# nianticlabs/map-free-reloc

Measured on AMD Instinct MI355X. Metric: image-pairs/sec @ 540x720 (SuperPoint+SuperGlue + PnP w/ depth), higher is better.
Workload: dtype f32 in / f32 accumulate; matrix products of the 3x3 convolutions, attention, the transformer's linear layers and SuperPoint's 1x1 descriptor head on the f16 matrix cores with every fp32 operand carried as TWO f16 terms (xh = rne_f16(x), xl = rne_f16((x - xh) 2^11); weights pre-scaled per output feat

## Files before the change

include/mfr_hip.h:

```cpp
#ifndef MFR_HIP_H
#define MFR_HIP_H
#include <stddef.h>
#include <stdint.h>

#ifdef __cplusplus
extern "C" {
#endif

#define MFR_ABI_VERSION 6

#define MFR_K_F32 0
#define MFR_K_F64 1

#define MFR_E_ARG      (-1)
#define MFR_E_LAUNCH   (-2)
#define MFR_E_WORKSPACE (-3)

#define MFR_ST_OK          0
#define MFR_ST_TOO_FEW     1
#define MFR_ST_BAD_DEPTH   2
#define MFR_ST_NO_MODEL    3
#define MFR_ST_DEGENERATE  4

int mfr_abi_version(void);
// ... 193 lines not shown
int mfr_sift_detect(const uint8_t *gray, int B, int H, int W, int nfeatures, int Nmax, int cand_cap, void *workspace,
                    size_t workspace_bytes, float *kpts, float *desc, float *size, float *angle, float *response,
                    int32_t *octave, int32_t *n, int32_t *status, void *stream);

size_t mfr_jpeg_workspace_bytes(int n, int H, int W, long long max_record_bytes, int subseq_bits);
int mfr_jpeg_decode(const void *headers, const uint8_t *records, const long long *offsets, int n, int H, int W,
                    long long max_record_bytes, float *gray, uint8_t *rgb, int32_t *status, int32_t *rounds, void *workspace,
                    size_t workspace_bytes, int subseq_bits, void *stream);

int mfr_resize_gray_bilinear(const uint8_t *rgb, int n, int H, int W, const int32_t *status,
                             const int32_t *y0, const int32_t *y1, const float *fy,
                             const int32_t *x0, const int32_t *x1, const float *fx,
                             int h, int w, float *out, void *stream);

size_t mfr_wino_f16x2_filter_bytes(int Cin, int Cout);
int mfr_wino_f16x2_filter_transform(const float *w, int Cin, int Cout, void *upk, void *stream);
int mfr_conv3x3_wino_f16x2(const float *x, const void *upk, const float *bias, const float *residual, int B, int Cin, int Cout,
                           int H, int W, int act, int pool, float *y, void *stream);
size_t mfr_conv3x3_direct_f16x2_filter_bytes(int Cin, int Cout);
int mfr_conv3x3_direct_f16x2_filter_pack(const float *w, int Cin, int Cout, void *packed, void *stream);
int mfr_conv3x3_direct_f16x2(const float *x, const void *packed, const float *bias, const float *residual, int B, int Cin, int Cout,
                             int H, int W, int act, int pool, float *y, void *stream);
int mfr_conv3x3_direct_f16x2_rows(const float *x, const void *packed, const float *bias, int B, int Cin, int Cout, int H, int W, int act, float *yrows, int ldy, void *stream);
int mfr_conv3x3s2_direct_f16x2(const float *x, const void *packed, const float *bias, int B, int Cin, int Cout, int H, int W, int act, float *y, void *stream);
int mfr_sp_conv1ab_f16x2(const float *gray, const float *w1a, const float *b1a, const void *upk1b, const float *bias1b, int B, int H, int W, float *y, void *stream);
size_t mfr_wino_bf16x3_filter_bytes(int Cin, int Cout);
int mfr_wino_bf16x3_filter_transform(const float *w, int Cin, int Cout, void *upk, void *stream);
int mfr_conv3x3_wino_bf16x3(const float *x, const void *upk, const float *bias, const float *residual, int B, int Cin, int Cout,
                            int H, int W, int act, int pool, float *y, void *stream);
size_t mfr_wino_filter_bytes(int Cin, int Cout);
int mfr_wino_filter_transform(const float *w, int Cin, int Cout, float *upk, void *stream);
int mfr_conv3x3_wino(const float *x, const float *upk, const float *bias, const float *residual, int B, int Cin, int Cout,
                     int H, int W, int act, int pool, float *y, void *stream);
int mfr_conv3x3_wino_variant(const float *x, const float *upk, const float *bias, const float *residual, int B, int Cin, int Cout,
                             int H, int W, int act, int pool, int variant, float *y, void *stream);

int mfr_corr_warp_fwd(const float *q, const float *k, const float *v, const float *grid, int B, int Dq, int N,
                      float *warped, float *pos, float *max_score, float *row_max, float *row_sum, void *stream);
int mfr_corr_warp_bwd(const float *q, const float *k, const float *v, const float *grid, int B, int Dq, int N,
                      const float *d_warped, const float *d_pos, const float *d_max, const float *delta,
                      const float *row_max, const float *row_sum, float *dq, float *dk, float *dv, void *stream);

#ifdef __cplusplus
}
#endif
#endif
// ... 1 lines not shown
```

map-free-reloc_amd/_lib.py:

```python
import ctypes as C
import os

_HERE = os.path.dirname(os.path.abspath(__file__))
SO_PATH = os.path.join(_HERE, "csrc", "libmfr_hip.so")

_lib = None

_vp, _i, _d, _u64, _sz = C.c_void_p, C.c_int, C.c_double, C.c_uint64, C.c_size_t

SIGNATURES = {
    "mfr_abi_version": (_i, []),
    "mfr_target_arch": (C.c_char_p, []),
    "mfr_f16x2_guard_bind": (_i, [_vp]),
    "mfr_test_f64_ops": (_i, [_vp, _vp, _vp, _i, _vp, _vp]),
    "mfr_test_sample": (_i, [_u64, _vp, _i, _i, _i, _i, _vp, _vp]),
    "mfr_pnp_workspace_bytes": (_sz, [_i, _i, _i]),
    "mfr_pnp_solve_batch": (_i, [_vp, _vp, _vp, _i, _i, _vp, _i, _i, _vp, _vp, _i, _i, _d, _d, _u64, _vp,
                                 _vp, _sz, _vp, _vp, _vp, _vp, _vp, _vp]),
    "mfr_depth_min": (_i, [_vp, _i, _i, _i, _vp, _vp]),
    "mfr_pnp_lift": (_i, [_vp, _vp, _vp, _i, _i, _vp, _vp, _i, _i, _vp, _i, _vp, _vp, _vp, _vp, _vp]),
    "mfr_pnp_ransac": (_i, [_vp, _vp, _vp, _i, _i, _vp, _i, _i, _d, _d, _u64, _vp, _vp, _vp, _vp, _vp, _vp, _vp,
                            _vp, _vp, _vp, _vp]),
    "mfr_emat_workspace_bytes": (_sz, [_i, _i, _i]),
    "mfr_magsac_lut": (_i, [_vp, _i]),
# ... 39 lines not shown
    "mfr_loftr_ot_match_workspace_bytes": (_sz, [_i, _i, _i]),
    "mfr_loftr_ot_match": (_i, [_vp, _i, _i, _i, _i, _i, C.c_float, _i, C.c_float, _i, _vp, _sz, _vp, _vp, _vp, _vp, _vp, _vp, _i, _vp]),
    "mfr_loftr_coarse_match_variant": (_i, [_vp, _i, _i, _i, _i, _i, C.c_float, C.c_float, _i, _vp, _sz, _vp, _vp, _vp, _vp, _i, _vp]),
    "mfr_loftr_fine_attention": (_i, [_vp, _i, _vp, _vp, _i, _i, _i, _i, _i, _vp, _i, _vp]),
    "mfr_loftr_gather_windows": (_i, [_vp, _i, _i, _i, _i, _vp, _vp, _i, _i, _i, _i, _vp, _vp]),
    "mfr_loftr_fine_match": (_i, [_vp, _vp, _i, _i, _i, _i, C.c_float, _vp, _vp, _vp, _vp, _vp]),
    "mfr_conv3x3_c1_relu": (_i, [_vp, _vp, _vp, _i, _i, _i, _i, _vp, _vp]),
    "mfr_bias_relu_nchw": (_i, [_vp, _vp, _i, _i, _i, _vp]),
    "mfr_conv1x1_nchw": (_i, [_vp, _vp, _vp, _i, _i, _i, _i, _vp, _vp]),
    "mfr_nchw_to_rows": (_i, [_vp, _vp, _i, _i, _i, _i, _vp, C.c_longlong, _i, _vp]),
    "mfr_bias_pool2_relu_nchw": (_i, [_vp, _vp, _i, _i, _i, _i, _vp, _vp]),
    "mfr_wino_bf16x3_filter_bytes": (_sz, [_i, _i]),
    "mfr_wino_bf16x3_filter_transform": (_i, [_vp, _i, _i, _vp, _vp]),
    "mfr_conv3x3_wino_bf16x3": (_i, [_vp, _vp, _vp, _vp, _i, _i, _i, _i, _i, _i, _i, _vp, _vp]),
    "mfr_sp_conv1ab_f16x2": (_i, [_vp, _vp, _vp, _vp, _vp, _i, _i, _i, _vp, _vp]),
    "mfr_wino_f16x2_filter_bytes": (_sz, [_i, _i]),
    "mfr_wino_f16x2_filter_transform": (_i, [_vp, _i, _i, _vp, _vp]),
    "mfr_conv3x3_wino_f16x2": (_i, [_vp, _vp, _vp, _vp, _i, _i, _i, _i, _i, _i, _i, _vp, _vp]),
    "mfr_conv3x3_direct_f16x2_filter_bytes": (_sz, [_i, _i]),
    "mfr_conv3x3_direct_f16x2_filter_pack": (_i, [_vp, _i, _i, _vp, _vp]),
    "mfr_conv3x3_direct_f16x2": (_i, [_vp, _vp, _vp, _vp, _i, _i, _i, _i, _i, _i, _i, _vp, _vp]),
    "mfr_conv3x3s2_direct_f16x2": (_i, [_vp, _vp, _vp, _i, _i, _i, _i, _i, _i, _vp, _vp]),
    "mfr_conv3x3_direct_f16x2_rows": (_i, [_vp, _vp, _vp, _i, _i, _i, _i, _i, _i, _vp, _i, _vp]),
    "mfr_wino_filter_bytes": (_sz, [_i, _i]),
    "mfr_wino_filter_transform": (_i, [_vp, _i, _i, _vp, _vp]),
    "mfr_conv3x3_wino": (_i, [_vp, _vp, _vp, _vp, _i, _i, _i, _i, _i, _i, _i, _vp, _vp]),
    "mfr_conv3x3_wino_variant": (_i, [_vp, _vp, _vp, _vp, _i, _i, _i, _i, _i, _i, _i, _i, _vp, _vp]),
    "mfr_layernorm": (_i, [_vp, _i, _vp, _vp, _vp, _i, C.c_longlong, _i, C.c_float, _vp, _i, _vp]),
    "mfr_conv_gemm_bf16": (_i, [_vp, C.c_longlong, _vp, _vp, C.c_longlong, _vp, _i, _i, _i, _vp, _vp, C.c_longlong, _i,
                                _i, _i, _i, _vp, _vp, _vp, _vp, _vp]),
    "mfr_conv_pack_nhwc_halo": (_i, [_vp, _i, _i, _i, _i, _i, _i, _vp, _i, _vp]),
    "mfr_conv_unpack_nchw": (_i, [_vp, _i, _i, _i, _i, _i, _vp, _vp]),
    "mfr_conv_pack_cm_halo": (_i, [_vp, _i, C.c_longlong, _i, _i, _i, C.c_longlong, _i, _i, C.c_longlong, _vp, _vp]),
    "mfr_upsample2x_add": (_i, [_vp, _vp, _i, _i, _i, _vp]),
    "mfr_upsample_bilinear": (_i, [_vp, _vp, _i, _i, _i, _i, _i, _i, _vp]),
    "mfr_corr_warp_fwd": (_i, [_vp, _vp, _vp, _vp, _i, _i, _i, _vp, _vp, _vp, _vp, _vp, _vp]),
    "mfr_corr_warp_bwd": (_i, [_vp, _vp, _vp, _vp, _i, _i, _i, _vp, _vp, _vp, _vp, _vp, _vp, _vp, _vp, _vp, _vp]),
    "mfr_kabsch_fwd": (_i, [_vp, _i, _vp, _vp]),
    "mfr_kabsch_bwd": (_i, [_vp, _vp, _i, _vp, _vp]),
    "mfr_rootsift": (_i, [_vp, _i, _vp, _vp, _vp]),
    "mfr_desc_ratio_match": (_i, [_vp, _vp, _vp, _vp, _vp, _vp, _i, _i, _i, _vp, _vp, _d, _vp, _vp, _vp, _vp, _i, _vp, _vp]),
    "mfr_sift_workspace_bytes": (_sz, [_i, _i, _i, _i]),
    "mfr_sift_level_offset": (C.c_longlong, [_i, _i, _i, _i, _i, _vp, _vp]),
    "mfr_sift_blur_taps": (_i, [_i, _vp, _vp]),
    "mfr_sift_detect": (_i, [_vp, _i, _i, _i, _i, _i, _i, _vp, _sz, _vp, _vp, _vp, _vp, _vp, _vp, _vp, _vp, _vp]),
    "mfr_jpeg_workspace_bytes": (_sz, [_i, _i, _i, C.c_longlong, _i]),
# ... 55 lines not shown
```

map-free-reloc_amd/csrc/conv_direct.hip:

```cpp
#include <hip/hip_runtime.h>
#include <stdint.h>
#include <type_traits>

#include "../../include/mfr_hip.h"
#include "wave_dev.h"
#include "split_f16.h"
#include "guard.h"

using namespace mfr;

typedef float dc_f32x16 __attribute__((ext_vector_type(16)));
#define DC_OOB 0x80000000u
#define DC_PC 34
#define DC_FRAGS_PER_TAP 6
#ifndef DC_NW
#define DC_NW 4
#endif

#ifdef DC_PROF
__device__ unsigned long long dc_prof[8][64];
#define DC_STAMP(k) do { if (blockIdx.x == (gridDim.x / 2 | 5u) && lane == 0) { __builtin_amdgcn_sched_barrier(0); dc_prof[w][(k)] = __builtin_amdgcn_s_memtime(); __builtin_amdgcn_sched_barrier(0); } } while (0)
extern "C" int *mfr_guard_current(void) { return nullptr; }
#else
#define DC_STAMP(k) do { } while (0)
#endif

#define DC_IC(k) std::integral_constant<int, k>{}
template <int MG, int NW, int STR> struct DcGeom {
    static constexpr int NT = 64 * NW;
    static constexpr int NGW = NW / MG;
    static constexpr int TR = 4 * NGW;
    static constexpr int PR = STR == 1 ? TR + 2 : 2 * TR + 1;
    static constexpr int PCW = STR == 1 ? DC_PC : 66;
    static constexpr int P = PR * PCW;
    static constexpr int PPAD = (P + 63) / 64 * 64;
    static constexpr int STAGE = 4 * PPAD;
    static constexpr int R = (2 * PPAD + NT - 1) / NT;
};

__global__ void __launch_bounds__(64) dc_scale_kernel(const float *__restrict__ w, int Cin, int Cout, int cpad, float *__restrict__ oscale)
{
    const int co = blockIdx.x, lane = threadIdx.x;
    float mx = 0.f;
    if (co < Cout)
        for (int t = lane; t < Cin * 9; t += 64) mx = fmaxf(mx, fabsf(w[(size_t)co * Cin * 9 + t]));
    mx = wave_max(mx);
    if (lane == 0 && co < cpad) oscale[co] = 1.0f / sf_feature_scale(mx);
}
__global__ void __launch_bounds__(256) dc_pack_kernel(const float *__restrict__ w, int Cin, int Cout, int nks, long long total, const float *__restrict__ oscale, uint4 *__restrict__ out)
{
    const long long t = (long long)blockIdx.x * 256 + threadIdx.x;
    if (t >= total) return;
    const int l = (int)(t & 63);
    long long f = t >> 6;
    const int term = (int)(f % 3); f /= 3;
    const int m = (int)(f & 1); f >>= 1;
    const int tap = (int)(f % 9); f /= 9;
    const int c = (int)(f % nks);
    const int cg = (int)(f / nks);
    const int co = cg * 64 + m * 32 + (l & 31);
    const float s = 1.0f / oscale[co];
    unsigned short hw[8];
#pragma unroll
    for (int e = 0; e < 8; ++e) {
        const int ci = 16 * c + 8 * (l >> 5) + e;
        const float v = (co < Cout && ci < Cin) ? w[((size_t)co * Cin + ci) * 9 + tap] * s : 0.f;
        unsigned short wh, wl, wq;
        sf_split_w(v, wh, wl, wq);
        hw[e] = term == 0 ? wh : term == 1 ? wl : wq;
    }
    out[t] = make_uint4((unsigned)hw[0] | ((unsigned)hw[1] << 16), (unsigned)hw[2] | ((unsigned)hw[3] << 16),
                        (unsigned)hw[4] | ((unsigned)hw[5] << 16), (unsigned)hw[6] | ((unsigned)hw[7] << 16));
}

template <int MG, int NW, bool POOL, int STR>
__global__ void __launch_bounds__(64 * NW, 8 / NW) conv_direct_f16x2_kernel(
    const float *__restrict__ x, const uint4 *__restrict__ wp, unsigned wp_bytes, const float *__restrict__ oscale, const float *__restrict__ bias,
    const float *__restrict__ residual, float *__restrict__ y, int Cin, int Cout, int H, int W, int nbx, int nby, int S, int ncgw, int nks, int act, int *guard, int ldrows)
{
    static_assert(STR == 1 || (STR == 2 && !POOL), "stride 1 or 2; no pooled strided variant");
    using G = DcGeom<MG, NW, STR>;
    __shared__ __attribute__((aligned(16))) uint4 lds[2 * G::STAGE];
    const int tid = threadIdx.x, lane = tid & 63;
    const int w = __builtin_amdgcn_readfirstlane(tid >> 6);
    const int xcd = blockIdx.x & 7, slot = blockIdx.x >> 3;
    const int cgi = slot % ncgw, s = (slot / ncgw) * 8 + xcd;
    if (s >= S) return;
    const int bx = s % nbx, by = (s / nbx) % nby, b = s / (nbx * nby);
    const int x0 = 32 * bx, y0 = G::TR * by;
    const int HW = H * W;
    const int Hout = STR == 1 ? H : (H - 1) / 2 + 1, Wout = STR == 1 ? W : (W - 1) / 2 + 1;
    const bool tail = !POOL && NW == 4 && MG == 2 && cgi == ncgw - 1 && (Cout - cgi * 128 + 31) / 32 == 3;

    const __amdgpu_buffer_rsrc_t rsX = __builtin_amdgcn_make_buffer_rsrc((void *)(x + (size_t)b * Cin * HW), 0, Cin * HW * 4, MFR_RSRC_FLAGS);
    unsigned voff[G::R];
    int wdst[G::R], hh[G::R];
#pragma unroll
    for (int r = 0; r < G::R; ++r) {
        const int h = (G::NT * r + 64 * w) / G::PPAD;
        const int p = G::NT * r + tid - h * G::PPAD;
        const int pr = p / G::PCW, q = p - pr * G::PCW;
        const int pc = STR == 1 ? q : 2 * (q % 33) + q / 33;
        const int gy = STR * y0 - 1 + pr, gx = STR * x0 - 1 + pc;
        const bool ok = h < 2 && p < G::P && pc < STR * 32 + 3 - STR && gy >= 0 && gy < H && gx >= 0 && gx < W;
        voff[r] = ok ? (unsigned)(gy * W + gx) * 4u : DC_OOB;
        hh[r] = h < 2 ? h : 0;
        wdst[r] = h < 2 ? h * G::PPAD + p : G::P + (lane & 15);
    }
    float sv[8];
    auto sload = [&](int r, int c) {
#pragma unroll
        for (int e = 0; e < 8; ++e) {
            const int ch = 16 * c + 8 * hh[r] + e;
            sv[e] = __builtin_bit_cast(float, __builtin_amdgcn_raw_buffer_load_b32(rsX, ch < Cin ? voff[r] : DC_OOB, (unsigned)ch * (unsigned)HW * 4u, 0));
        }
    };
    auto swrite = [&](int r, int buf) {
        unsigned h[4], l[4];
#pragma unroll
        for (int k = 0; k < 4; ++k) sf_split2(sv[2 * k], sv[2 * k + 1], SF_LOW_SCALE, h[k], l[k]);
        lds[buf * G::STAGE + wdst[r]] = make_uint4(h[0], h[1], h[2], h[3]);
        lds[buf * G::STAGE + 2 * G::PPAD + wdst[r]] = make_uint4(l[0], l[1], l[2], l[3]);
    };

    const __amdgpu_buffer_rsrc_t rsW = __builtin_amdgcn_make_buffer_rsrc((void *)wp, 0, (int)wp_bytes, MFR_RSRC_FLAGS);
    const unsigned lane16 = (unsigned)lane * 16u;
    auto body = [&](auto mbc, auto nbc) {
    constexpr int MB = decltype(mbc)::value, NB = decltype(nbc)::value;
    const int mg = MB == 2 ? w % MG : 0, ng = MB == 2 ? w / MG : w;
    const int mb0 = (cgi * MG + mg) * 2;
    const unsigned kstride = (unsigned)nks * (9u * DC_FRAGS_PER_TAP * 1024u);
    auto aload = [&](int c, int tap, int m, int term) -> uint4 {
        const int mbg = mb0 + m;
        return __builtin_bit_cast(uint4, __builtin_amdgcn_raw_buffer_load_b128(rsW, lane16, (unsigned)(mbg >> 1) * kstride + (unsigned)(((c * 9 + tap) * 2 + (mbg & 1)) * 3 + term) * 1024u, 0));
    };
    const int rdb = (lane >> 5) * G::PPAD + (STR * NB * ng) * G::PCW + (lane & 31);
    auto tapoff = [](int n, int dy, int dx) { return STR == 1 ? (n + dy) * G::PCW + dx : (2 * n + dy) * G::PCW + (dx & 1) * 33 + (dx >> 1); };

    DC_STAMP(0);
    {
        float pv[G::R][8];
#pragma unroll
        for (int r = 0; r < G::R; ++r) { sload(r, 0);
#pragma unroll
            for (int e = 0; e < 8; ++e) pv[r][e] = sv[e]; }
#pragma unroll
        for (int r = 0; r < G::R; ++r) {
#pragma unroll
            for (int e = 0; e < 8; ++e) sv[e] = pv[r][e];
            swrite(r, 0); }
    }
    uint4 AE[MB][3], AO[MB][3], Bh[NB], Bl[NB];
#pragma unroll
    for (int m = 0; m < MB; ++m) { AE[m][0] = aload(0, 0, m, 0); AE[m][1] = aload(0, 0, m, 1); AE[m][2] = aload(0, 0, m, 2); AO[m][1] = aload(0, 1, m, 1); AO[m][2] = aload(0, 1, m, 2); AO[m][0] = AE[m][0]; }
    dc_f32x16 acc[MB][NB];
#pragma unroll
    for (int m = 0; m < MB; ++m)
#pragma unroll
        for (int n = 0; n < NB; ++n)
#pragma unroll
            for (int r = 0; r < 16; ++r) acc[m][n][r] = 0.f;

#define DC_SL(r) (G::R == 5 ? 5 * (r) : 8 * (r))
#define DC_SW(r) (G::R == 5 ? ((r) == 4 ? 26 : 5 * (r) + 4) : ((r) == 2 ? 24 : 8 * (r) + 6))
    DC_STAMP(1);
    for (int c = 0; c < nks; ++c) {
        DC_STAMP(2 + 4 * (c & 7));
        __syncthreads();
        const uint4 *st = lds + (c & 1) * G::STAGE + rdb;
        const int nbuf = (c + 1) & 1;
#pragma unroll
        for (int n = 0; n < NB; ++n) Bl[n] = st[2 * G::PPAD + tapoff(n, 0, 0)];
        DC_STAMP(3 + 4 * (c & 7));
        auto stage_event = [&](int phi) {
#pragma unroll
            for (int r = 0; r < G::R; ++r) {
                if (phi == DC_SW(r)) swrite(r, nbuf);
                if (phi == DC_SL(r)) sload(r, c + 1);
            }
        };
        auto do_tap = [&](auto tapc, uint4 (&A)[MB][3], uint4 (&Ao)[MB][3]) {
            constexpr int tap = decltype(tapc)::value;
            constexpr int dy = tap / 3, dx = tap - 3 * dy;
            constexpr int dyn = (tap + 1) / 3, dxn = (tap + 1) - 3 * dyn;
#pragma unroll
            for (int n = 0; n < NB; ++n) Bh[n] = st[tapoff(n, dy, dx)];
            __builtin_amdgcn_sched_barrier(0);
#pragma unroll
            for (int m = 0; m < MB; ++m) Ao[m][0] = aload(c, tap + 1, m, 0);
            stage_event(3 * tap);
#pragma unroll
            for (int m = 0; m < MB; ++m)
#pragma unroll
                for (int n = 0; n < NB; ++n) acc[m][n] = SF_MFMA(A[m][2], Bl[n], acc[m][n]);
            __builtin_amdgcn_sched_barrier(0);
#pragma unroll
            for (int m = 0; m < MB; ++m) A[m][2] = aload(c, tap + 2, m, 2);
            if (tap < 8) {
#pragma unroll
                for (int n = 0; n < NB; ++n) Bl[n] = st[2 * G::PPAD + tapoff(n, dyn, dxn)];
            }
            stage_event(3 * tap + 1);
#pragma unroll
            for (int m = 0; m < MB; ++m)
#pragma unroll
                for (int n = 0; n < NB; ++n) acc[m][n] = SF_MFMA(A[m][1], Bh[n], acc[m][n]);
            __builtin_amdgcn_sched_barrier(0);
#pragma unroll
            for (int m = 0; m < MB; ++m) A[m][1] = aload(c, tap + 2, m, 1);
            stage_event(3 * tap + 2);
#pragma unroll
            for (int m = 0; m < MB; ++m)
#pragma unroll
                for (int n = 0; n < NB; ++n) acc[m][n] = SF_MFMA(A[m][0], Bh[n], acc[m][n]);
            __builtin_amdgcn_sched_barrier(0);
        };
        do_tap(DC_IC(0), AE, AO); do_tap(DC_IC(1), AO, AE); do_tap(DC_IC(2), AE, AO); DC_STAMP(4 + 4 * (c & 7)); do_tap(DC_IC(3), AO, AE); do_tap(DC_IC(4), AE, AO);
        do_tap(DC_IC(5), AO, AE); DC_STAMP(5 + 4 * (c & 7)); do_tap(DC_IC(6), AE, AO); do_tap(DC_IC(7), AO, AE); do_tap(DC_IC(8), AE, AO);
#pragma unroll
        for (int m = 0; m < MB; ++m)
#pragma unroll
            for (int t = 0; t < 3; ++t) { const uint4 tmp = AE[m][t]; AE[m][t] = AO[m][t]; AO[m][t] = tmp; }
    }
#undef DC_SL
#undef DC_SW

    const int H = Hout, W = Wout, HW = Hout * Wout;
    DC_STAMP(34);
    float gchk = 0.f;
    if (guard) {
#pragma unroll
        for (int m = 0; m < MB; ++m)
#pragma unroll
            for (int n = 0; n < NB; ++n)
#pragma unroll
                for (int r = 0; r < 16; ++r) MFR_GUARD_ACC(gchk, acc[m][n][r]);
        mfr_guard_commit(guard, gchk);
    }
    const int px = x0 + (lane & 31);
    const int half = lane >> 5;
    const int Ho = POOL ? (H >> 1) : H, Wo = POOL ? (W >> 1) : W;
    const size_t cstride = (size_t)Ho * Wo;
    const int cpad1 = (Cout + 63) / 64 * 64 - 1;
    auto activate = [&](float v) { return act == 1 ? fmaxf(v, 0.f) : act == 2 ? (v > 0.f ? v : 0.01f * v) : v; };
    const __amdgpu_buffer_rsrc_t rsY = __builtin_amdgcn_make_buffer_rsrc((void *)(y + (size_t)b * Cout * cstride), 0, (int)(Cout * cstride * 4), MFR_RSRC_FLAGS);
    const __amdgpu_buffer_rsrc_t rsR = __builtin_amdgcn_make_buffer_rsrc((void *)(residual ? residual + (size_t)b * Cout * HW : nullptr), 0, residual ? Cout * HW * 4 : 0, MFR_RSRC_FLAGS);
    if (ldrows > 0) {
        const __amdgpu_buffer_rsrc_t rsQ = __builtin_amdgcn_make_buffer_rsrc((void *)(y + (size_t)b * HW * ldrows), 0, HW * ldrows * 4, MFR_RSRC_FLAGS);
        unsigned pixrow[NB];
#pragma unroll
        for (int n = 0; n < NB; ++n) {
            const int oy = y0 + NB * ng + n;
            pixrow[n] = (oy < H && px < W) ? (unsigned)(oy * W + px) * (unsigned)ldrows * 4u : DC_OOB;
        }
        DC_STAMP(36);
#pragma unroll
        for (int m = 0; m < MB; ++m)
#pragma unroll
            for (int q = 0; q < 4; ++q) {
                const int c0 = (mb0 + m) * 32 + 8 * q + 4 * half;
                float o4[4], b4[4];
#pragma unroll
                for (int k = 0; k < 4; ++k) { o4[k] = oscale[min(c0 + k, cpad1)]; b4[k] = bias ? bias[min(c0 + k, Cout - 1)] : 0.f; }
                const unsigned cpart = c0 < Cout ? (unsigned)c0 * 4u : 0x40000000u;
#pragma unroll
                for (int n = 0; n < NB; ++n) {
                    typedef unsigned dc_u32x4 __attribute__((ext_vector_type(4)));
                    const float4 v = make_float4(activate(__builtin_fmaf(acc[m][n][4 * q], o4[0], b4[0])), activate(__builtin_fmaf(acc[m][n][4 * q + 1], o4[1], b4[1])),
                                                 activate(__builtin_fmaf(acc[m][n][4 * q + 2], o4[2], b4[2])), activate(__builtin_fmaf(acc[m][n][4 * q + 3], o4[3], b4[3])));
                    __builtin_amdgcn_raw_buffer_store_b128(__builtin_bit_cast(dc_u32x4, v), rsQ, cpart + pixrow[n], 0, 0);
                }
            }
    } else if (!(W & 3)) {
        const int L8 = lane >> 3, L7 = lane & 7;
        float os[MB][4], bv[MB][4];
        unsigned cho[MB][4];
#pragma unroll
        for (int m = 0; m < MB; ++m)
#pragma unroll
            for (int j = 0; j < 4; ++j) {
                const int co = (mb0 + m) * 32 + 8 * j + L8;
                os[m][j] = oscale[min(co, cpad1)];
                bv[m][j] = bias ? bias[min(co, Cout - 1)] : 0.f;
                cho[m][j] = co < Cout ? (unsigned)co * (unsigned)cstride * 4u : 0x40000000u;
            }
        unsigned pix[NB];
#pragma unroll
        for (int n = 0; n < NB; ++n) {
            const int oy = y0 + NB * ng + n, xg = x0 + 4 * L7;
            if (POOL) pix[n] = ((oy >> 1) < Ho && (xg >> 1) < Wo) ? (unsigned)((oy >> 1) * Wo + (xg >> 1)) * 4u : DC_OOB;
            else      pix[n] = (oy < H && xg < W) ? (unsigned)(oy * W + xg) * 4u : DC_OOB;
        }
        __syncthreads();
        DC_STAMP(36);
        float *tb = (float *)lds + 1024 * w;
        constexpr int NSTEP = POOL ? 2 : 1;
        constexpr int DC_RD = 6;
        float4 rv[POOL ? 1 : MB * NB * 4];
        auto rload = [&](int it) {
            if (!POOL) rv[it] = __builtin_bit_cast(float4, __builtin_amdgcn_raw_buffer_load_b128(rsR, cho[it / (4 * NB)][it & 3] + pix[(it >> 2) % NB], 0, 0));
        };
        if (!POOL && residual) {
#pragma unroll
            for (int it = 0; it < DC_RD; ++it) rload(it);
        }
#pragma unroll
        for (int m = 0; m < MB; ++m)
#pragma unroll
            for (int n = 0; n < NB; n += NSTEP) {
                if (m == 1 && n == 0) DC_STAMP(37);
#pragma unroll
                for (int r = 0; r < 16; ++r)
// ... 12 lines not shown
                        if (residual) {
                            if (it + DC_RD < MB * NB * 4) rload(it + DC_RD);
                            v.x += rv[it].x; v.y += rv[it].y; v.z += rv[it].z; v.w += rv[it].w;
                        }
                        v = make_float4(activate(v.x), activate(v.y), activate(v.z), activate(v.w));
                        typedef unsigned dc_u32x4 __attribute__((ext_vector_type(4)));
                        __builtin_amdgcn_raw_buffer_store_b128(__builtin_bit_cast(dc_u32x4, v), rsY, cho[m][j] + pix[n], 0, 0);
                    }
                }
            }
    } else {
        float osv[MB][16], bvv[MB][16];
#pragma unroll
        for (int m = 0; m < MB; ++m)
#pragma unroll
            for (int r = 0; r < 16; ++r) {
                const int co = (mb0 + m) * 32 + (r & 3) + 8 * (r >> 2) + 4 * half;
                osv[m][r] = oscale[min(co, cpad1)];
                bvv[m][r] = bias ? bias[min(co, Cout - 1)] : 0.f;
            }
        unsigned pixoff[NB];
#pragma unroll
        for (int n = 0; n < NB; ++n) {
            const int oy = y0 + NB * ng + n;
            if (POOL) pixoff[n] = (!(lane & 1) && (oy >> 1) < Ho && (px >> 1) < Wo) ? (unsigned)((oy >> 1) * Wo + (px >> 1)) * 4u : DC_OOB;
            else      pixoff[n] = (oy < H && px < W) ? (unsigned)(oy * W + px) * 4u : DC_OOB;
        }
        auto choff = [&](int m, int r) -> unsigned {
            const int co = (mb0 + m) * 32 + (r & 3) + 8 * (r >> 2) + 4 * half;
            return co < Cout ? (unsigned)co * (unsigned)cstride * 4u : 0x40000000u;
        };
        DC_STAMP(36);
        if (POOL) {
#pragma unroll
            for (int m = 0; m < MB; ++m)
#pragma unroll
                for (int r = 0; r < 16; ++r) {
                    const unsigned co4 = choff(m, r);
#pragma unroll
                    for (int n = 0; n < NB; n += 2) {
                        float v = fmaxf(__builtin_fmaf(acc[m][n][r], osv[m][r], bvv[m][r]), __builtin_fmaf(acc[m][n + 1][r], osv[m][r], bvv[m][r]));
                        v = activate(fmaxf(v, __shfl_xor(v, 1)));
                        __builtin_amdgcn_raw_buffer_store_b32(__builtin_bit_cast(unsigned, v), rsY, co4 + pixoff[n], 0, 0);
                    }
                }
        } else {
            constexpr int DC_RD = 4;
// ... 46 lines not shown
    return n;
}
int mfr_dconv_profile(unsigned long long *out_host)
{
    return hipMemcpyFromSymbol(out_host, HIP_SYMBOL(dc_prof), sizeof(unsigned long long) * 512, 0, hipMemcpyDeviceToHost) == hipSuccess ? 0 : MFR_E_LAUNCH;
}
#endif

size_t mfr_conv3x3_direct_f16x2_filter_bytes(int Cin, int Cout) { return (Cin <= 0 || Cout <= 0) ? 0 : dc_frag_bytes(Cin, Cout) + (size_t)((Cout + 63) / 64) * 64 * 4; }

int mfr_conv3x3_direct_f16x2_filter_pack(const float *w, int Cin, int Cout, void *packed, void *stream)
{
    if (!w || !packed || Cin <= 0 || Cout <= 0) return MFR_E_ARG;
    const size_t fb = dc_frag_bytes(Cin, Cout);
    const long long total = (long long)(fb / 16);
    float *oscale = (float *)((char *)packed + fb);
    const int cpad = (Cout + 63) / 64 * 64;
    hipLaunchKernelGGL(dc_scale_kernel, dim3((unsigned)cpad), dim3(64), 0, (hipStream_t)stream, w, Cin, Cout, cpad, oscale);
    hipLaunchKernelGGL(dc_pack_kernel, dim3((unsigned)((total + 255) / 256)), dim3(256), 0, (hipStream_t)stream, w, Cin, Cout, (Cin + 15) / 16, total, (const float *)oscale, (uint4 *)packed);
    CHECK_LAUNCH();
    return 0;
}

static int dc_conv(const float *x, const void *packed, const float *bias, const float *residual, int B, int Cin, int Cout, int H, int W,
                   int act, int pool, float *y, int ldrows, void *stream)
{
    if (!x || !packed || !y || B <= 0 || Cin <= 0 || Cout <= 0 || H <= 0 || W <= 0 || act < 0 || act > 2) return MFR_E_ARG;
    if (pool && (H < 2 || W < 2 || residual)) return MFR_E_ARG;
    if ((size_t)4 * (Cin + 15) * H * W >= 0x7fffffffull || (size_t)4 * Cout * H * W >= 0x40000000ull) return MFR_E_ARG;
    const size_t fb = dc_frag_bytes(Cin, Cout);
    if (fb >= 0x7fffffffull) return MFR_E_ARG;
    const int nks = (Cin + 15) / 16;
    const float *oscale = (const float *)((const char *)packed + fb);
    const int mg = Cout > 64 ? 2 : 1;
    const int tr = 4 * DC_NW / mg;
    const int nbx = (W + 31) / 32, nby = (H + tr - 1) / tr, ncgw = (Cout + 64 * mg - 1) / (64 * mg);
    const long long S = (long long)nbx * nby * B;
    const long long grid = ((S + 7) / 8) * 8 * ncgw;
    if (grid > 0x7fffffffll) return MFR_E_ARG;
    hipStream_t st = (hipStream_t)stream;
    int *guard = mfr_guard_current();
#define DC_LAUNCH(MGV, POOLV) hipLaunchKernelGGL((conv_direct_f16x2_kernel<MGV, DC_NW, POOLV, 1>), dim3((unsigned)grid), dim3(64 * DC_NW), 0, st, x, (const uint4 *)packed, (unsigned)fb, oscale, bias, \
                                                  residual, y, Cin, Cout, H, W, nbx, nby, (int)S, ncgw, nks, act, guard, ldrows)
    if (mg == 1) { if (pool) DC_LAUNCH(1, true); else DC_LAUNCH(1, false); }
    else         { if (pool) DC_LAUNCH(2, true); else DC_LAUNCH(2, false); }
#undef DC_LAUNCH
    CHECK_LAUNCH();
    return 0;
}

int mfr_conv3x3_direct_f16x2(const float *x, const void *packed, const float *bias, const float *residual, int B, int Cin, int Cout, int H, int W,
                             int act, int pool, float *y, void *stream)
{
    return dc_conv(x, packed, bias, residual, B, Cin, Cout, H, W, act, pool, y, 0, stream);
}

int mfr_conv3x3_direct_f16x2_rows(const float *x, const void *packed, const float *bias, int B, int Cin, int Cout, int H, int W, int act, float *yrows, int ldy, void *stream)
{
    if (ldy < Cout || (ldy & 3) || (Cout & 3) || H <= 0 || W <= 0 || (size_t)4 * ldy * H * W >= 0x40000000ull) return MFR_E_ARG;
    return dc_conv(x, packed, bias, nullptr, B, Cin, Cout, H, W, act, 0, yrows, ldy, stream);
}

int mfr_conv3x3s2_direct_f16x2(const float *x, const void *packed, const float *bias, int B, int Cin, int Cout, int H, int W, int act, float *y, void *stream)
{
    if (!x || !packed || !y || B <= 0 || Cin <= 0 || Cout <= 0 || H <= 0 || W <= 0 || act < 0 || act > 2) return MFR_E_ARG;
    const int Ho = (H - 1) / 2 + 1, Wo = (W - 1) / 2 + 1;
    if ((size_t)4 * (Cin + 15) * H * W >= 0x7fffffffull || (size_t)4 * Cout * Ho * Wo >= 0x40000000ull) return MFR_E_ARG;
    const size_t fb = dc_frag_bytes(Cin, Cout);
    if (fb >= 0x7fffffffull) return MFR_E_ARG;
    const int nks = (Cin + 15) / 16;
    const float *oscale = (const float *)((const char *)packed + fb);
    const int nbx = (Wo + 31) / 32, nby = (Ho + 3) / 4, ncgw = (Cout + 255) / 256;
    const long long S = (long long)nbx * nby * B;
    const long long grid = ((S + 7) / 8) * 8 * ncgw;
    if (grid > 0x7fffffffll) return MFR_E_ARG;
    hipLaunchKernelGGL((conv_direct_f16x2_kernel<4, 4, false, 2>), dim3((unsigned)grid), dim3(256), 0, (hipStream_t)stream, x, (const uint4 *)packed, (unsigned)fb, oscale, bias,
                       (const float *)nullptr, y, Cin, Cout, H, W, nbx, nby, (int)S, ncgw, nks, act, mfr_guard_current(), 0);
    CHECK_LAUNCH();
    return 0;
}

}
```

map-free-reloc_amd/nets/conv.py:

```python
import torch

from .. import _lib, options

WASTE_LIMIT = {"bf16x3": 0.2, "f16x2": 0.5}


def prefer_split(H, W, split=None):
    mode = options.get("CONV_KERNEL")
    if mode in ("split", "direct"):
        return True
    if mode == "exact":
        return False
    tiles = (W + 1) // 2
    return (-(-tiles // 16) * 16) / tiles - 1.0 <= WASTE_LIMIT[split or options.get("SPLIT")]


class WinoConv3x3:

    def __init__(self, weight, bias, split=None):
        lib = _lib.load(require_gpu=True)
        self.split = split or options.get("SPLIT")
        if self.split not in ("f16x2", "bf16x3"):
            raise ValueError(f"WinoConv3x3: unknown split {self.split!r}")
        self.w, self.b = weight.contiguous(), bias
# ... 23 lines not shown
            if self.split != "f16x2":
                raise ValueError("CONV_KERNEL = 'direct' exists in the f16x2 arithmetic only")
            self.direct = DirectConv3x3(self.w, self.b)
        return self.direct

    def __call__(self, x, act=0, pool=False, residual=None):
        lib = _lib.load()
        mode = options.get("CONV_KERNEL")
        if mode == "direct" or (mode == "auto" and self.split == "f16x2"):
            return self._direct()(x, act=act, pool=pool, residual=residual)
        x = x.contiguous()
        B, C, H, W = x.shape
        y = torch.empty((B, self.co, H // 2, W // 2) if pool else (B, self.co, H, W), dtype=torch.float32, device=x.device)
        res = _lib.ptr(residual.contiguous()) if residual is not None else None
        if self.u_exact is None or prefer_split(H, W, self.split):
            _lib.check(self._conv_split(_lib.ptr(x), _lib.ptr(self.u_split), _lib.ptr(self.b), res, B, C, self.co, H, W, int(act), int(pool),
                                        _lib.ptr(y), _lib.stream_ptr()), f"mfr_conv3x3_wino_{self.split}")
        else:
            _lib.check(lib.mfr_conv3x3_wino(_lib.ptr(x), _lib.ptr(self.u_exact), _lib.ptr(self.b), res, B, C, self.co, H, W, int(act), int(pool),
                                            _lib.ptr(y), _lib.stream_ptr()), "mfr_conv3x3_wino")
        return y


class DirectConv3x3:

    def __init__(self, weight, bias):
        lib = _lib.load(require_gpu=True)
        self.w, self.b = weight.contiguous().float(), bias
        self.co, self.ci = int(weight.shape[0]), int(weight.shape[1])
        self.split = "f16x2"
        self.packed = torch.empty(lib.mfr_conv3x3_direct_f16x2_filter_bytes(self.ci, self.co), dtype=torch.uint8, device=weight.device)
        _lib.check(lib.mfr_conv3x3_direct_f16x2_filter_pack(_lib.ptr(self.w), self.ci, self.co, _lib.ptr(self.packed), _lib.stream_ptr()),
                   "mfr_conv3x3_direct_f16x2_filter_pack")

    def rows(self, x, act=0):
        lib = _lib.load()
        x = x.contiguous()
        B, C, H, W = x.shape
        assert C == self.ci and x.dtype == torch.float32 and self.co % 4 == 0
        y = torch.empty(B, H, W, self.co, dtype=torch.float32, device=x.device)
        _lib.check(lib.mfr_conv3x3_direct_f16x2_rows(_lib.ptr(x), _lib.ptr(self.packed), _lib.ptr(self.b), B, C, self.co, H, W, int(act), _lib.ptr(y), self.co,
                                                     _lib.stream_ptr()), "mfr_conv3x3_direct_f16x2_rows")
        return y

    def strided(self, x, act=0):
        lib = _lib.load()
        x = x.contiguous()
        B, C, H, W = x.shape
        assert C == self.ci and x.dtype == torch.float32
        y = torch.empty(B, self.co, (H - 1) // 2 + 1, (W - 1) // 2 + 1, dtype=torch.float32, device=x.device)
        _lib.check(lib.mfr_conv3x3s2_direct_f16x2(_lib.ptr(x), _lib.ptr(self.packed), _lib.ptr(self.b), B, C, self.co, H, W, int(act), _lib.ptr(y), _lib.stream_ptr()),
                   "mfr_conv3x3s2_direct_f16x2")
        return y

    def __call__(self, x, act=0, pool=False, residual=None):
        lib = _lib.load()
        x = x.contiguous()
        B, C, H, W = x.shape
        assert C == self.ci and x.dtype == torch.float32
        y = torch.empty((B, self.co, H // 2, W // 2) if pool else (B, self.co, H, W), dtype=torch.float32, device=x.device)
        res = _lib.ptr(residual.contiguous()) if residual is not None else None
        _lib.check(lib.mfr_conv3x3_direct_f16x2(_lib.ptr(x), _lib.ptr(self.packed), _lib.ptr(self.b), res, B, C, self.co, H, W, int(act), int(pool),
                                                _lib.ptr(y), _lib.stream_ptr()), "mfr_conv3x3_direct_f16x2")
        return y


class IgemmConv:

    def __init__(self, weight, bias, stride=1, padding=None):
        lib = _lib.load(require_gpu=True)
        co, ci, kh, kw = (int(v) for v in weight.shape)
        self.co, self.ci, self.kh, self.kw = co, ci, kh, kw
        self.stride, self.pad = int(stride), (kh // 2 if padding is None else int(padding))
        K = lib.mfr_conv_igemm_k(ci, kh, kw)
        w = weight.detach().float()
        if ci == 1:
            m = torch.zeros(co, K, dtype=torch.float32, device=w.device)
            m[:, :kh * kw] = w.reshape(co, kh * kw)
        else:
            cpad = K // (kh * kw)
            m = torch.zeros(co, kh * kw, cpad, dtype=torch.float32, device=w.device)
            m[:, :, :ci] = w.permute(0, 2, 3, 1).reshape(co, kh * kw, ci)
            m = m.reshape(co, K)
        nb = lib.mfr_gemm_f16x2_pack_bytes(co, K)
# ... 24 lines not shown
```

map-free-reloc_amd/options.py:

```python
_SPEC = {
    "SPLIT": ("f16x2", ("f16x2", "bf16x3")),
    "CONV": ("wino", ("wino", "miopen")),
    "CONV_KERNEL": ("auto", ("auto", "split", "exact", "direct")),
    "FUSED_CONV1": (True, (False, True)),
    "FUSED_CONV_RELU": (False, (False, True)),
    "RPR_CONV": ("hip", ("hip", "miopen")),
    "RPR_CONV_BWD": ("lib", ("lib", "hip")),
    "RPR_CONV_ORDER": ("tap_inner", ("tap_inner", "tap_outer")),
    "RPR_WGRAD_SPLITS": (16, None),
    "RPR_ENCODER_NHWC": (False, (False, True)),
}
_VALUES = {k: v[0] for k, v in _SPEC.items()}
_EXPLICIT = set()


def names():
    return sorted(_SPEC)


def default(name):
    return _SPEC[name][0]


def get(name):
    return _VALUES[name]

# ... 54 lines not shown
```

Measured before the change: 1297.

## Add linearized pixel-strip tiling to direct f16x2 3x3 conv for narrow images

Adds a 'linear' tile geometry to the direct 3x3 conv kernel. The image is treated as a flattened padded-pitch strip, and each block covers 256 consecutive output pixels rather than 32-wide column tiles. The aim is to cut wasted lanes and halo overhead when the width is slightly above a multiple of 32 (65-80, 129-144), where the column tiling leaves most of a tile empty. An auto heuristic selects it for Cout > 64 without pooling. The cost is a pad column per row, extra index divisions, and masking of the guard checksum for padded pixels.

```diff
diff --git a/include/mfr_hip.h b/include/mfr_hip.h
--- a/include/mfr_hip.h
+++ b/include/mfr_hip.h
@@ -239,6 +239,8 @@
 int mfr_conv3x3_direct_f16x2(const float *x, const void *packed, const float *bias, const float *residual, int B, int Cin, int Cout,
                              int H, int W, int act, int pool, float *y, void *stream);
 int mfr_conv3x3_direct_f16x2_rows(const float *x, const void *packed, const float *bias, int B, int Cin, int Cout, int H, int W, int act, float *yrows, int ldy, void *stream);
+int mfr_conv3x3_direct_f16x2_tiled(const float *x, const void *packed, const float *bias, const float *residual, int B, int Cin, int Cout, int H, int W,
+                                   int act, int pool, float *y, int ldrows, int tile_mode, int pitch, void *stream);
 int mfr_conv3x3s2_direct_f16x2(const float *x, const void *packed, const float *bias, int B, int Cin, int Cout, int H, int W, int act, float *y, void *stream);
 int mfr_sp_conv1ab_f16x2(const float *gray, const float *w1a, const float *b1a, const void *upk1b, const float *bias1b, int B, int H, int W, float *y, void *stream);
 size_t mfr_wino_bf16x3_filter_bytes(int Cin, int Cout);
diff --git a/map-free-reloc_amd/_lib.py b/map-free-reloc_amd/_lib.py
--- a/map-free-reloc_amd/_lib.py
+++ b/map-free-reloc_amd/_lib.py
@@ -85,6 +85,7 @@
     "mfr_conv3x3_direct_f16x2": (_i, [_vp, _vp, _vp, _vp, _i, _i, _i, _i, _i, _i, _i, _vp, _vp]),
     "mfr_conv3x3s2_direct_f16x2": (_i, [_vp, _vp, _vp, _i, _i, _i, _i, _i, _i, _vp, _vp]),
     "mfr_conv3x3_direct_f16x2_rows": (_i, [_vp, _vp, _vp, _i, _i, _i, _i, _i, _i, _vp, _i, _vp]),
+    "mfr_conv3x3_direct_f16x2_tiled": (_i, [_vp, _vp, _vp, _vp, _i, _i, _i, _i, _i, _i, _i, _vp, _i, _i, _i, _vp]),
     "mfr_wino_filter_bytes": (_sz, [_i, _i]),
     "mfr_wino_filter_transform": (_i, [_vp, _i, _i, _vp, _vp]),
     "mfr_conv3x3_wino": (_i, [_vp, _vp, _vp, _vp, _i, _i, _i, _i, _i, _i, _i, _vp, _vp]),
diff --git a/map-free-reloc_amd/csrc/conv_direct.hip b/map-free-reloc_amd/csrc/conv_direct.hip
--- a/map-free-reloc_amd/csrc/conv_direct.hip
+++ b/map-free-reloc_amd/csrc/conv_direct.hip
@@ -26,14 +26,15 @@
 #endif
 
 #define DC_IC(k) std::integral_constant<int, k>{}
-template <int MG, int NW, int STR> struct DcGeom {
+#define DC_LT 256
+template <int MG, int NW, int STR, int LIN = 0> struct DcGeom {
     static constexpr int NT = 64 * NW;
     static constexpr int NGW = NW / MG;
     static constexpr int TR = 4 * NGW;
     static constexpr int PR = STR == 1 ? TR + 2 : 2 * TR + 1;
     static constexpr int PCW = STR == 1 ? DC_PC : 66;
     static constexpr int P = PR * PCW;
-    static constexpr int PPAD = (P + 63) / 64 * 64;
+    static constexpr int PPAD = LIN ? LIN : (P + 63) / 64 * 64;
     static constexpr int STAGE = 4 * PPAD;
     static constexpr int R = (2 * PPAD + NT - 1) / NT;
 };
@@ -73,13 +74,15 @@
                         (unsigned)hw[4] | ((unsigned)hw[5] << 16), (unsigned)hw[6] | ((unsigned)hw[7] << 16));
 }
 
-template <int MG, int NW, bool POOL, int STR>
+template <int MG, int NW, bool POOL, int STR, int LIN = 0>
 __global__ void __launch_bounds__(64 * NW, 8 / NW) conv_direct_f16x2_kernel(
     const float *__restrict__ x, const uint4 *__restrict__ wp, unsigned wp_bytes, const float *__restrict__ oscale, const float *__restrict__ bias,
-    const float *__restrict__ residual, float *__restrict__ y, int Cin, int Cout, int H, int W, int nbx, int nby, int S, int ncgw, int nks, int act, int *guard, int ldrows)
+    const float *__restrict__ residual, float *__restrict__ y, int Cin, int Cout, int H, int W, int nbx, int nby, int S, int ncgw, int nks, int act, int *guard, int ldrows,
+    int Pw)
 {
     static_assert(STR == 1 || (STR == 2 && !POOL), "stride 1 or 2; no pooled strided variant");
-    using G = DcGeom<MG, NW, STR>;
+    static_assert(LIN == 0 || (MG == 2 && NW == 4 && !POOL && STR == 1 && LIN % 64 == 0), "linear geometry: MG = 2, stride 1, no pooling");
+    using G = DcGeom<MG, NW, STR, LIN>;
     __shared__ __attribute__((aligned(16))) uint4 lds[2 * G::STAGE];
     const int tid = threadIdx.x, lane = tid & 63;
     const int w = __builtin_amdgcn_readfirstlane(tid >> 6);
@@ -88,6 +91,7 @@
     if (s >= S) return;
     const int bx = s % nbx, by = (s / nbx) % nby, b = s / (nbx * nby);
     const int x0 = 32 * bx, y0 = G::TR * by;
+    const int u0 = DC_LT * bx;
     const int HW = H * W;
     const int Hout = STR == 1 ? H : (H - 1) / 2 + 1, Wout = STR == 1 ? W : (W - 1) / 2 + 1;
     const bool tail = !POOL && NW == 4 && MG == 2 && cgi == ncgw - 1 && (Cout - cgi * 128 + 31) / 32 == 3;
@@ -99,6 +103,16 @@
     for (int r = 0; r < G::R; ++r) {
         const int h = (G::NT * r + 64 * w) / G::PPAD;
         const int p = G::NT * r + tid - h * G::PPAD;
+        if constexpr (LIN > 0) {
+            const int il = G::NT * r + tid - (h < 2 ? 0 : 128), hl = (G::NT * r + 64 * w - (h < 2 ? 0 : 128)) / G::PPAD, pl = il - hl * G::PPAD;
+            const int U = u0 - Pw - 1 + pl;
+            const int yy = (int)((unsigned)max(U, 0) / (unsigned)Pw), xx = max(U, 0) - yy * Pw;
+            const bool ok = pl < DC_LT + 2 + 2 * Pw && U >= 0 && yy < H && xx < W;
+            voff[r] = ok ? (unsigned)(yy * W + xx) * 4u : DC_OOB;
+            hh[r] = hl;
+            wdst[r] = il;
+            continue;
+        }
         const int pr = p / G::PCW, q = p - pr * G::PCW;
         const int pc = STR == 1 ? q : 2 * (q % 33) + q / 33;
         const int gy = STR * y0 - 1 + pr, gx = STR * x0 - 1 + pc;
@@ -134,8 +148,8 @@
         const int mbg = mb0 + m;
         return __builtin_bit_cast(uint4, __builtin_amdgcn_raw_buffer_load_b128(rsW, lane16, (unsigned)(mbg >> 1) * kstride + (unsigned)(((c * 9 + tap) * 2 + (mbg & 1)) * 3 + term) * 1024u, 0));
     };
-    const int rdb = (lane >> 5) * G::PPAD + (STR * NB * ng) * G::PCW + (lane & 31);
-    auto tapoff = [](int n, int dy, int dx) { return STR == 1 ? (n + dy) * G::PCW + dx : (2 * n + dy) * G::PCW + (dx & 1) * 33 + (dx >> 1); };
+    const int rdb = (lane >> 5) * G::PPAD + (LIN ? 32 * NB * ng : (STR * NB * ng) * G::PCW) + (lane & 31);
+    auto tapoff = [](int n, int dy, int dx) { return LIN ? 32 * n + dx : STR == 1 ? (n + dy) * G::PCW + dx : (2 * n + dy) * G::PCW + (dx & 1) * 33 + (dx >> 1); };
 
     DC_STAMP(0);
     {
@@ -161,16 +175,17 @@
 #pragma unroll
             for (int r = 0; r < 16; ++r) acc[m][n][r] = 0.f;
 
-#define DC_SL(r) (G::R == 5 ? 5 * (r) : 8 * (r))
-#define DC_SW(r) (G::R == 5 ? ((r) == 4 ? 26 : 5 * (r) + 4) : ((r) == 2 ? 24 : 8 * (r) + 6))
+#define DC_SL(r) (G::R == 5 ? 5 * (r) : G::R == 4 ? 6 * (r) : 8 * (r))
+#define DC_SW(r) (G::R == 5 ? ((r) == 4 ? 26 : 5 * (r) + 4) : G::R == 4 ? 6 * (r) + 5 : ((r) == 2 ? 24 : 8 * (r) + 6))
     DC_STAMP(1);
     for (int c = 0; c < nks; ++c) {
         DC_STAMP(2 + 4 * (c & 7));
         __syncthreads();
         const uint4 *st = lds + (c & 1) * G::STAGE + rdb;
+        const uint4 *const strow[3] = {st, LIN ? st + Pw : st, LIN ? st + 2 * Pw : st};
         const int nbuf = (c + 1) & 1;
 #pragma unroll
-        for (int n = 0; n < NB; ++n) Bl[n] = st[2 * G::PPAD + tapoff(n, 0, 0)];
+        for (int n = 0; n < NB; ++n) Bl[n] = strow[0][2 * G::PPAD + tapoff(n, 0, 0)];
         DC_STAMP(3 + 4 * (c & 7));
         auto stage_event = [&](int phi) {
 #pragma unroll
@@ -184,7 +199,7 @@
             constexpr int dy = tap / 3, dx = tap - 3 * dy;
             constexpr int dyn = (tap + 1) / 3, dxn = (tap + 1) - 3 * dyn;
 #pragma unroll
-            for (int n = 0; n < NB; ++n) Bh[n] = st[tapoff(n, dy, dx)];
+            for (int n = 0; n < NB; ++n) Bh[n] = strow[dy][tapoff(n, dy, dx)];
             __builtin_amdgcn_sched_barrier(0);
 #pragma unroll
             for (int m = 0; m < MB; ++m) Ao[m][0] = aload(c, tap + 1, m, 0);
@@ -198,7 +213,7 @@
             for (int m = 0; m < MB; ++m) A[m][2] = aload(c, tap + 2, m, 2);
             if (tap < 8) {
 #pragma unroll
-                for (int n = 0; n < NB; ++n) Bl[n] = st[2 * G::PPAD + tapoff(n, dyn, dxn)];
+                for (int n = 0; n < NB; ++n) Bl[n] = strow[dyn % 3][2 * G::PPAD + tapoff(n, dyn, dxn)];
             }
             stage_event(3 * tap + 1);
 #pragma unroll
@@ -227,17 +242,26 @@
 
     const int H = Hout, W = Wout, HW = Hout * Wout;
     DC_STAMP(34);
+    auto opix = [&](int n, int lp, int &oy, int &ox) {
+        const int u = u0 + 32 * (NB * ng + n) + lp; oy = (int)((unsigned)u / (unsigned)Pw); ox = u - oy * Pw;
+    };
     float gchk = 0.f;
     if (guard) {
+        bool real[NB];
+#pragma unroll
+        for (int n = 0; n < NB; ++n) {
+            real[n] = true;
+            if constexpr (LIN > 0) { int oy, ox; opix(n, lane & 31, oy, ox); real[n] = oy < H && ox < W; }
+        }
 #pragma unroll
         for (int m = 0; m < MB; ++m)
 #pragma unroll
             for (int n = 0; n < NB; ++n)
 #pragma unroll
-                for (int r = 0; r < 16; ++r) MFR_GUARD_ACC(gchk, acc[m][n][r]);
+                for (int r = 0; r < 16; ++r) MFR_GUARD_ACC(gchk, LIN > 0 && !real[n] ? 0.f : acc[m][n][r]);
         mfr_guard_commit(guard, gchk);
     }
-    const int px = x0 + (lane & 31);
+    const int px0 = x0 + (lane & 31);
     const int half = lane >> 5;
     const int Ho = POOL ? (H >> 1) : H, Wo = POOL ? (W >> 1) : W;
     const size_t cstride = (size_t)Ho * Wo;
@@ -250,7 +274,8 @@
         unsigned pixrow[NB];
 #pragma unroll
         for (int n = 0; n < NB; ++n) {
-            const int oy = y0 + NB * ng + n;
+            int oy = y0 + NB * ng + n, px = px0;
+            if constexpr (LIN > 0) opix(n, lane & 31, oy, px);
             pixrow[n] = (oy < H && px < W) ? (unsigned)(oy * W + px) * (unsigned)ldrows * 4u : DC_OOB;
         }
         DC_STAMP(36);
@@ -271,7 +296,7 @@
                     __builtin_amdgcn_raw_buffer_store_b128(__builtin_bit_cast(dc_u32x4, v), rsQ, cpart + pixrow[n], 0, 0);
                 }
             }
-    } else if (!(W & 3)) {
+    } else if (!(W & 3) && (LIN == 0 || !(Pw & 3))) {
         const int L8 = lane >> 3, L7 = lane & 7;
         float os[MB][4], bv[MB][4];
         unsigned cho[MB][4];
@@ -287,7 +312,8 @@
         unsigned pix[NB];
 #pragma unroll
         for (int n = 0; n < NB; ++n) {
-            const int oy = y0 + NB * ng + n, xg = x0 + 4 * L7;
+            int oy = y0 + NB * ng + n, xg = x0 + 4 * L7;
+            if constexpr (LIN > 0) opix(n, 4 * L7, oy, xg);
             if (POOL) pix[n] = ((oy >> 1) < Ho && (xg >> 1) < Wo) ? (unsigned)((oy >> 1) * Wo + (xg >> 1)) * 4u : DC_OOB;
             else      pix[n] = (oy < H && xg < W) ? (unsigned)(oy * W + xg) * 4u : DC_OOB;
         }
@@ -346,7 +372,8 @@
         unsigned pixoff[NB];
 #pragma unroll
         for (int n = 0; n < NB; ++n) {
-            const int oy = y0 + NB * ng + n;
+            int oy = y0 + NB * ng + n, px = px0;
+            if constexpr (LIN > 0) opix(n, lane & 31, oy, px);
             if (POOL) pixoff[n] = (!(lane & 1) && (oy >> 1) < Ho && (px >> 1) < Wo) ? (unsigned)((oy >> 1) * Wo + (px >> 1)) * 4u : DC_OOB;
             else      pixoff[n] = (oy < H && px < W) ? (unsigned)(oy * W + px) * 4u : DC_OOB;
         }
@@ -439,8 +466,18 @@
     return 0;
 }
 
+static bool dc_lin_auto(int W, int Cout, int ldrows)
+{
+    if (Cout <= 64) return false;
+    if (W >= 65 && W <= 80) return true;
+    if (W >= 129 && W <= 144) return ldrows == 0;
+    return false;
+}
+#define DC_LIN_AUTO(W, Cout, ldrows) dc_lin_auto(W, Cout, ldrows)
+#define DC_LIN_PW_SMALL ((448 - DC_LT - 2) / 2)
+#define DC_LIN_PW_LARGE ((576 - DC_LT - 2) / 2)
 static int dc_conv(const float *x, const void *packed, const float *bias, const float *residual, int B, int Cin, int Cout, int H, int W,
-                   int act, int pool, float *y, int ldrows, void *stream)
+                   int act, int pool, float *y, int ldrows, int tile_mode, int pitch, void *stream)
 {
     if (!x || !packed || !y || B <= 0 || Cin <= 0 || Cout <= 0 || H <= 0 || W <= 0 || act < 0 || act > 2) return MFR_E_ARG;
     if (pool && (H < 2 || W < 2 || residual)) return MFR_E_ARG;
@@ -451,16 +488,29 @@
     const float *oscale = (const float *)((const char *)packed + fb);
     const int mg = Cout > 64 ? 2 : 1;
     const int tr = 4 * DC_NW / mg;
-    const int nbx = (W + 31) / 32, nby = (H + tr - 1) / tr, ncgw = (Cout + 64 * mg - 1) / (64 * mg);
+    if (tile_mode < 0 || tile_mode > 2 || pitch < 0) return MFR_E_ARG;
+    const bool lin_ok = DC_NW == 4 && mg == 2 && !pool && W + 1 <= DC_LIN_PW_LARGE;
+    if (tile_mode == 0) tile_mode = (lin_ok && DC_LIN_AUTO(W, Cout, ldrows)) ? 2 : 1;
+    int nbx = (W + 31) / 32, nby = (H + tr - 1) / tr;
+    const int ncgw = (Cout + 64 * mg - 1) / (64 * mg);
+    if (tile_mode == 2) {
+        if (!pitch) pitch = W + 1;
+        if (!lin_ok || pitch < W + 1 || pitch > DC_LIN_PW_LARGE) return MFR_E_ARG;
+        nbx = (int)(((long long)H * pitch + DC_LT - 1) / DC_LT), nby = 1;
+    }
     const long long S = (long long)nbx * nby * B;
     const long long grid = ((S + 7) / 8) * 8 * ncgw;
     if (grid > 0x7fffffffll) return MFR_E_ARG;
     hipStream_t st = (hipStream_t)stream;
     int *guard = mfr_guard_current();
-#define DC_LAUNCH(MGV, POOLV) hipLaunchKernelGGL((conv_direct_f16x2_kernel<MGV, DC_NW, POOLV, 1>), dim3((unsigned)grid), dim3(64 * DC_NW), 0, st, x, (const uint4 *)packed, (unsigned)fb, oscale, bias, \
-                                                  residual, y, Cin, Cout, H, W, nbx, nby, (int)S, ncgw, nks, act, guard, ldrows)
-    if (mg == 1) { if (pool) DC_LAUNCH(1, true); else DC_LAUNCH(1, false); }
-    else         { if (pool) DC_LAUNCH(2, true); else DC_LAUNCH(2, false); }
+#define DC_LAUNCH(MGV, POOLV, LINV) hipLaunchKernelGGL((conv_direct_f16x2_kernel<MGV, DC_NW, POOLV, 1, LINV>), dim3((unsigned)grid), dim3(64 * DC_NW), 0, st, x, (const uint4 *)packed, (unsigned)fb, oscale, bias, \
+                                                        residual, y, Cin, Cout, H, W, nbx, nby, (int)S, ncgw, nks, act, guard, ldrows, pitch)
+#if DC_NW == 4
+    if (tile_mode == 2) { if (pitch <= DC_LIN_PW_SMALL) DC_LAUNCH(2, false, 448); else DC_LAUNCH(2, false, 576); }
+    else
+#endif
+    if (mg == 1) { if (pool) DC_LAUNCH(1, true, 0); else DC_LAUNCH(1, false, 0); }
+    else         { if (pool) DC_LAUNCH(2, true, 0); else DC_LAUNCH(2, false, 0); }
 #undef DC_LAUNCH
     CHECK_LAUNCH();
     return 0;
@@ -469,13 +519,20 @@
 int mfr_conv3x3_direct_f16x2(const float *x, const void *packed, const float *bias, const float *residual, int B, int Cin, int Cout, int H, int W,
                              int act, int pool, float *y, void *stream)
 {
-    return dc_conv(x, packed, bias, residual, B, Cin, Cout, H, W, act, pool, y, 0, stream);
+    return dc_conv(x, packed, bias, residual, B, Cin, Cout, H, W, act, pool, y, 0, 0, 0, stream);
+}
+
+int mfr_conv3x3_direct_f16x2_tiled(const float *x, const void *packed, const float *bias, const float *residual, int B, int Cin, int Cout, int H, int W,
+                                   int act, int pool, float *y, int ldrows, int tile_mode, int pitch, void *stream)
+{
+    if (ldrows < 0 || (ldrows > 0 && (ldrows < Cout || (ldrows & 3) || (Cout & 3) || pool || residual || H <= 0 || W <= 0 || (size_t)4 * ldrows * H * W >= 0x40000000ull))) return MFR_E_ARG;
+    return dc_conv(x, packed, bias, residual, B, Cin, Cout, H, W, act, pool, y, ldrows, tile_mode, pitch, stream);
 }
 
 int mfr_conv3x3_direct_f16x2_rows(const float *x, const void *packed, const float *bias, int B, int Cin, int Cout, int H, int W, int act, float *yrows, int ldy, void *stream)
 {
     if (ldy < Cout || (ldy & 3) || (Cout & 3) || H <= 0 || W <= 0 || (size_t)4 * ldy * H * W >= 0x40000000ull) return MFR_E_ARG;
-    return dc_conv(x, packed, bias, nullptr, B, Cin, Cout, H, W, act, 0, yrows, ldy, stream);
+    return dc_conv(x, packed, bias, nullptr, B, Cin, Cout, H, W, act, 0, yrows, ldy, 0, 0, stream);
 }
 
 int mfr_conv3x3s2_direct_f16x2(const float *x, const void *packed, const float *bias, int B, int Cin, int Cout, int H, int W, int act, float *y, void *stream)
@@ -492,7 +549,7 @@
     const long long grid = ((S + 7) / 8) * 8 * ncgw;
     if (grid > 0x7fffffffll) return MFR_E_ARG;
     hipLaunchKernelGGL((conv_direct_f16x2_kernel<4, 4, false, 2>), dim3((unsigned)grid), dim3(256), 0, (hipStream_t)stream, x, (const uint4 *)packed, (unsigned)fb, oscale, bias,
-                       (const float *)nullptr, y, Cin, Cout, H, W, nbx, nby, (int)S, ncgw, nks, act, mfr_guard_current(), 0);
+                       (const float *)nullptr, y, Cin, Cout, H, W, nbx, nby, (int)S, ncgw, nks, act, mfr_guard_current(), 0, 0);
     CHECK_LAUNCH();
     return 0;
 }
diff --git a/map-free-reloc_amd/nets/conv.py b/map-free-reloc_amd/nets/conv.py
--- a/map-free-reloc_amd/nets/conv.py
+++ b/map-free-reloc_amd/nets/conv.py
@@ -69,7 +69,16 @@
         return y
 
 
+LINEAR_MAX_W = 158
+
+
 class DirectConv3x3:
+
+    def _tile_mode(self, W, pool):
+        tile = options.get("CONV_TILE")
+        if tile == "linear":
+            return 2 if (self.co > 64 and not pool and W <= LINEAR_MAX_W) else 1
+        return 1 if tile == "rows" else 0
 
     def __init__(self, weight, bias):
         lib = _lib.load(require_gpu=True)
@@ -86,6 +95,11 @@
         B, C, H, W = x.shape
         assert C == self.ci and x.dtype == torch.float32 and self.co % 4 == 0
         y = torch.empty(B, H, W, self.co, dtype=torch.float32, device=x.device)
+        mode = self._tile_mode(W, False)
+        if mode:
+            _lib.check(lib.mfr_conv3x3_direct_f16x2_tiled(_lib.ptr(x), _lib.ptr(self.packed), _lib.ptr(self.b), None, B, C, self.co, H, W, int(act), 0, _lib.ptr(y),
+                                                          self.co, mode, 0, _lib.stream_ptr()), "mfr_conv3x3_direct_f16x2_tiled")
+            return y
         _lib.check(lib.mfr_conv3x3_direct_f16x2_rows(_lib.ptr(x), _lib.ptr(self.packed), _lib.ptr(self.b), B, C, self.co, H, W, int(act), _lib.ptr(y), self.co,
                                                      _lib.stream_ptr()), "mfr_conv3x3_direct_f16x2_rows")
         return y
@@ -107,6 +121,11 @@
         assert C == self.ci and x.dtype == torch.float32
         y = torch.empty((B, self.co, H // 2, W // 2) if pool else (B, self.co, H, W), dtype=torch.float32, device=x.device)
         res = _lib.ptr(residual.contiguous()) if residual is not None else None
+        mode = self._tile_mode(W, pool)
+        if mode:
+            _lib.check(lib.mfr_conv3x3_direct_f16x2_tiled(_lib.ptr(x), _lib.ptr(self.packed), _lib.ptr(self.b), res, B, C, self.co, H, W, int(act), int(pool),
+                                                          _lib.ptr(y), 0, mode, 0, _lib.stream_ptr()), "mfr_conv3x3_direct_f16x2_tiled")
+            return y
         _lib.check(lib.mfr_conv3x3_direct_f16x2(_lib.ptr(x), _lib.ptr(self.packed), _lib.ptr(self.b), res, B, C, self.co, H, W, int(act), int(pool),
                                                 _lib.ptr(y), _lib.stream_ptr()), "mfr_conv3x3_direct_f16x2")
         return y
diff --git a/map-free-reloc_amd/options.py b/map-free-reloc_amd/options.py
--- a/map-free-reloc_amd/options.py
+++ b/map-free-reloc_amd/options.py
@@ -2,6 +2,7 @@
     "SPLIT": ("f16x2", ("f16x2", "bf16x3")),
     "CONV": ("wino", ("wino", "miopen")),
     "CONV_KERNEL": ("auto", ("auto", "split", "exact", "direct")),
+    "CONV_TILE": ("auto", ("auto", "rows", "linear")),
     "FUSED_CONV1": (True, (False, True)),
     "FUSED_CONV_RELU": (False, (False, True)),
     "RPR_CONV": ("hip", ("hip", "miopen")),
```

New measurement: 1332, median of 6. 2.7% higher.
